# earth-system-radiation/rte-ecckd

Hardware: AMD Instinct MI355X
Metric: Mcol*lay*gpt/s LW gas_optics+rte_lw (higher is better)
Workload: dtype f64

## Files before the change

### rte-ecckd_amd/__init__.py

```python
import ctypes as C
import os
import subprocess

import numpy as np

_HERE = os.path.dirname(os.path.abspath(__file__))
_CSRC = os.path.join(_HERE, "csrc")
LIB_PATH = os.environ.get("ECCKD_LIB", os.path.join(_HERE, "librte_ecckd_hip.so"))
HOST, DEVICE = 0, 1
MIXED = 2
NAME_LEN = 32

_SOURCES = ["kernels_gas_fused.hip", "kernels_tau.hip", "kernels_planck.hip", "kernels_rte_lw.hip", "kernels_rte_lw_split.hip",
            "kernels_rte_lw_jac.hip", "kernels_rte_lw_2str.hip",
            "kernels_rte_sw.hip", "kernels_rte_sw_sys.hip", "kernels_rte_gpt.hip", "kernels_optical_props.hip",
            "kernels_cloud_sampling.hip", "kernels_cloud_optics.hip",
            "capi.cpp", "nc_capi.cpp", "model.cpp", "cdf1.cpp"]
_HEADERS = ["kernels.hpp", "wave_pair.hpp", "sw_two_stream.hpp", "sw_two_stream_body.inc", "lw_two_stream.hpp", "lw_layer.hpp", "planck_at.hpp", "model.hpp", "cdf1.hpp", os.path.join("..", "..", "include", "ecckd_hip.h"),
            os.path.join("..", "..", "include", "ecckd_nc.h"), os.path.join("..", "..", "include", "rte_kernels_hip.h"),
            os.path.join("..", "..", "include", "rte_kernels_lw_2stream_hip.h")]
RTE_KERNELS_LIB = os.path.join(_HERE, "librte_kernels_hip.so")
_RTE_KERNELS_SRC = "rte_kernels_capi.cpp"
HIPCC_FLAGS = ["--offload-arch=gfx950", "-O3", "-std=c++17", "-fPIC", "-shared",
               "-ffp-contract=off", "-Wall", "-Wno-unused-function"]
# ... 189 lines not shown
            getattr(L, f).argtypes = [C.c_void_p, C.c_int, C.c_int] + [C.c_void_p] * 4 + [C.c_int] + [C.c_void_p] * 3 + [C.c_int, C.c_void_p]
    _lib = L
    return L


def last_error():
    return lib().ecckd_last_error().decode()


FAST, REFERENCE_ORDER = 0, 1


def set_arithmetic(mode):
    if lib().ecckd_set_arithmetic(int(mode)):
        raise ValueError(last_error())


def get_arithmetic():
    return lib().ecckd_get_arithmetic()


SOLVER_OPTIONS = ("lw_tau_thresh", "lw_series_terms", "lw_inc_flux_isotropic", "sw_k_floor", "sw_dir_clamp", "lw_solver",
                  "lw_split_seg", "gas_merge_scalars", "lw_tail_split", "sw_tail_split", "sw_solver", "gas_slab_f32",
                  "gas_tile_sync")


def set_solver_option(name, value):
    if lib().ecckd_set_solver_option(name.encode(), float(value)):
        raise ValueError(last_error())


def get_solver_option(name):
    v = C.c_double()
    if lib().ecckd_get_solver_option(name.encode(), C.byref(v)):
        raise ValueError(last_error())
    return v.value


def solver_options():
    out = {}
    for n in SOLVER_OPTIONS:
        try:
            out[n] = get_solver_option(n)
        except ValueError:
            if LIB_PATH == os.path.join(_HERE, "librte_ecckd_hip.so"):
                raise
    return out
# ... 1230 lines not shown
```

### rte-ecckd_amd/csrc/capi.cpp

```cpp
#include <hip/hip_runtime.h>

#include <atomic>
#include <cmath>
#include <cstdint>
#include <cstdlib>
#include <cstring>
#include <map>
#include <mutex>
#include <string>
#include <vector>

#include "../../include/ecckd_hip.h"
#include "kernels.hpp"
#include "model.hpp"

namespace {

thread_local std::string g_err;

int fail(const std::string &msg) {
  g_err = msg;
  return 1;
}
}
// ... 149 lines not shown

double gw(bool f32) {
  return f32 ? (double)(1.f / (9.80665f * 0.001f * 28.970f)) : 1. / ((double)9.80665f * (double)0.001f * (double)28.970f);
}
const double *table(const ecckd_model *m, size_t off, bool f32) {
  return f32 ? reinterpret_cast<const double *>(m->dbuf32 + off) : m->dbuf + off;
}

std::atomic<int> g_arith{0};

struct SolverOptions {
  std::atomic<double> lw_tau_thresh{0.};
  std::atomic<int> lw_series_terms{2};
  std::atomic<int> lw_inc_flux_isotropic{0};
  std::atomic<double> sw_k_floor{1.e-12};
  std::atomic<int> sw_dir_clamp{0};
  std::atomic<int> lw_solver{0};
  std::atomic<int> lw_split_seg{10};
  std::atomic<int> gas_merge_scalars{1};
  std::atomic<int> lw_tail_split{1};
  std::atomic<int> sw_tail_split{1};
  std::atomic<int> gas_slab_f32{2};
  std::atomic<int> gas_tile_sync{-1};
  std::atomic<int> sw_solver{0};
  std::atomic<int> lw_both_skies{1};
  std::atomic<int> lw_jac_inline{1};
};
SolverOptions g_opt;

double lw_tau_thresh(bool f32) {
  const double t = g_opt.lw_tau_thresh.load();
  return t > 0. ? t : (f32 ? std::sqrt(1.1920928955078125e-07) : std::sqrt(2.220446049250313e-16));
}

struct ProfRec { const char *name; hipEvent_t start, stop; };
std::mutex g_prof_mu;
bool g_prof_on = false;
std::vector<ProfRec> g_prof;

struct ProfScope {
  hipStream_t s;
  ProfRec r{};
  bool on;
  ProfScope(const char *name, hipStream_t stream) : s(stream), on(g_prof_on) {
    if (!on) return;
    r.name = name;
    if (hipEventCreate(&r.start) != hipSuccess || hipEventCreate(&r.stop) != hipSuccess) { on = false; return; }
    (void)hipEventRecord(r.start, s);
  }
  ~ProfScope() {
    if (!on) return;
// ... 124 lines not shown
    }
    if (fast) {
      fa.mode = (sw && last) ? 2 : 0;
      if (g_opt.gas_merge_scalars.load() && !f32) merge_scalar_gases(a, f32);
      const int nv_lut = a.lut >= 0 ? a.seq[a.lut].nv : 0;
      int pass_clamp = 0;
      for (int k = 0; k < a.nseq; ++k) pass_clamp |= a.seq[k].clamp;
      if (pl && first_pass && !sw &&
          fused_planck_rows(a.ng, a.np, a.nt, a.nbil, nv_lut, m->ntp, pass_clamp, f32) > 0) {
        fa.mode = 1;
        fa.ntp = m->ntp;
        fa.planck = table(m, m->off_planck, f32);
        fa.pt0 = m->temperature_planck[0];
        fa.pdt = m->temperature_planck[1] - m->temperature_planck[0];
        fa.tlev = pl->tlev; fa.tsfc = pl->tsfc;
        fa.lay_source = pl->lay_source; fa.lev_source_inc = pl->lev_inc;
        fa.lev_source_dec = pl->lev_dec; fa.sfc_source = pl->sfc_source;
        if (planck_done) *planck_done = true;
      }
      fa.f32 = f32;
      {
        const int sync = g_opt.gas_tile_sync.load();
        fa.tile_sync = sync >= 0 ? sync : (fa.mode != 0 ? 1 : 0);
      }
      ScratchLease flag_lease;
      fa.slab32 = (!f32 && !plan && m->f32_exact && fa.mode == 1) ? g_opt.gas_slab_f32.load() : 0;
      if (fa.slab32 == 2) fa.choose_buf = static_cast<int *>(stream_scratch_optional(m->device, stream, 256, flag_lease, g_flag_pool));
      if (f32 && ((fa.mode != 1 && fa.mode != 2) || !last || !first_pass))
        return fail("ecckd: single precision is implemented for one-pass gas optics (fused longwave, shortwave); this "
                    "model / gas list needs the multi-pass or unfused path");
      if (plan) {
        FusedPlan fp;
        HIPCHK(prepare_gas_fused(fa, fp));
        if (plan->npass == 0) { plan->first_fused = 1; plan->planck_fused = fa.mode == 1; plan->first = fp; }
        ++plan->npass;
      } else {
        ProfScope prof(fa.mode == 1 ? (f32 ? "gas_lw_fused_f32" : "gas_lw_fused") : "tau", stream);
        HIPCHK(launch_gas_fused(fa, stream));
      }
    } else {
      if (f32) return fail("ecckd: single precision needs the fast arithmetic mode (ecckd_set_arithmetic(0))");
      if (plan) {
        ++plan->npass;
      } else {
        ProfScope prof("tau", stream);
        HIPCHK(launch_tau(a, stream));
// ... 296 lines not shown
  else if (n == "lw_tail_split") g_opt.lw_tail_split.store(value != 0. ? 1 : 0);
  else if (n == "sw_tail_split") g_opt.sw_tail_split.store(value != 0. ? 1 : 0);
  else if (n == "sw_solver") {
    if (value != 0. && value != 1.) return fail("ecckd_set_solver_option: sw_solver must be 0 (layer-systolic) or 1 (two-pass per lane)");
    g_opt.sw_solver.store((int)value);
  }
  else if (n == "lw_both_skies") {
    if (value != 0. && value != 1.) return fail("ecckd_set_solver_option: lw_both_skies must be 0 (two launches) or 1 (dual-sky kernel)");
    g_opt.lw_both_skies.store((int)value);
  }
  else if (n == "lw_jac_inline") {
    if (value != 0. && value != 1.) return fail("ecckd_set_solver_option: lw_jac_inline must be 0 (stand-alone Jacobian kernel) or 1 (inside the layer-split kernel)");
    g_opt.lw_jac_inline.store((int)value);
  }
  else if (n == "gas_slab_f32") {
    if (value != 0. && value != 1. && value != 2.) return fail("ecckd_set_solver_option: gas_slab_f32 must be 0 (never), 1 (always) or 2 (auto)");
    g_opt.gas_slab_f32.store((int)value);
  }
  else if (n == "gas_tile_sync") {
    if (value != 0. && value != 1. && value != -1.)
      return fail("ecckd_set_solver_option: gas_tile_sync must be 0 (off), 1 (a block barrier per tile) or -1 (the default of each mode)");
    g_opt.gas_tile_sync.store((int)value);
  }
  else return fail("ecckd_set_solver_option: unknown option '" + n + "' (lw_tau_thresh, lw_series_terms, "
                   "lw_inc_flux_isotropic, sw_k_floor, sw_dir_clamp, lw_solver, lw_split_seg, gas_merge_scalars, lw_tail_split, "
                   "sw_tail_split, sw_solver, gas_slab_f32, gas_tile_sync, lw_both_skies, lw_jac_inline)");
  return 0;
}

int ecckd_get_solver_option(const char *name, double *value) {
  if (!name || !value) return fail("ecckd_get_solver_option: null argument");
  const std::string n(name);
  if (n == "lw_tau_thresh") *value = lw_tau_thresh(false);
  else if (n == "lw_series_terms") *value = g_opt.lw_series_terms.load();
  else if (n == "lw_inc_flux_isotropic") *value = g_opt.lw_inc_flux_isotropic.load();
  else if (n == "sw_k_floor") *value = g_opt.sw_k_floor.load();
  else if (n == "sw_dir_clamp") *value = g_opt.sw_dir_clamp.load();
  else if (n == "lw_solver") *value = g_opt.lw_solver.load();
  else if (n == "lw_split_seg") *value = g_opt.lw_split_seg.load();
  else if (n == "gas_merge_scalars") *value = g_opt.gas_merge_scalars.load();
  else if (n == "lw_tail_split") *value = g_opt.lw_tail_split.load();
  else if (n == "sw_tail_split") *value = g_opt.sw_tail_split.load();
  else if (n == "sw_solver") *value = g_opt.sw_solver.load();
  else if (n == "gas_slab_f32") *value = g_opt.gas_slab_f32.load();
  else if (n == "gas_tile_sync") *value = g_opt.gas_tile_sync.load();
  else if (n == "lw_both_skies") *value = g_opt.lw_both_skies.load();
  else if (n == "lw_jac_inline") *value = g_opt.lw_jac_inline.load();
  else return fail("ecckd_get_solver_option: unknown option '" + n + "'");
  return 0;
}

size_t ecckd_rte_lw_scratch_bytes(int ncol, int nlay, int ngpt) {
  return ncol > 0 && nlay > 0 ? ecckd::rte_lw_scratch_bytes(ncol, nlay, ngpt) : 0;
}
size_t ecckd_rte_sw_scratch_bytes(int ncol, int nlay, int ngpt) {
  return ncol > 0 && nlay > 0 ? ecckd::rte_sw_scratch_bytes(ncol, nlay, ngpt) : 0;
}

size_t ecckd_rte_sw_tail_scratch_bytes(int device, int ncol, int nlay, int ngpt) {
  if (ncol <= 0 || nlay <= 0 || ngpt <= 0 || device < 0 || device >= 16 || !g_opt.sw_tail_split.load()) return 0;
  ecckd::RteSwArgs a{};
  a.ncol = ncol; a.nlay = nlay; a.ng = ngpt;
  if (g_opt.sw_solver.load() == 0 && ecckd::rte_sw_sys_applies(a)) return ecckd::rte_sw_sys_plan(a, simd_slots(device) / 4);
  long first = -1;
  size_t at = 0;
  return ecckd::rte_sw_tail_plan(a, &first, &at);
}
static size_t sw_fluxes_solver_bytes(int device, int ncol, int nlay, int ngpt) {
// ... 2118 lines not shown
```

### rte-ecckd_amd/csrc/kernels.hpp

```cpp
#pragma once
#include <hip/hip_runtime.h>

namespace ecckd {

constexpr int kMaxSeq = 16;
constexpr int kTauPassGases = 10;
constexpr int kLdsBudget = 160 * 1024;

struct SeqGas {
  const double *coef;
  const double *vmr;
  long long cs, ls;
  double scalar;
  double ref;
  double mf0;
  double log_mf0;
  double d_log_vmr;
  int code;
  int nv;
  int slot;
  int clamp;
};

struct TauArgs {
// ... 20 lines not shown
  int seg;
};

struct UDiv { double d, r; int exact; };

struct SlotArgs {
  const double *vmr;
  long long ls;
  unsigned cs_bytes;
  double alpha, beta;
};

struct FusedArgs {
  TauArgs tau;
  UDiv ud_dlp, ud_dt, ud_dlv, ud_pdt;
  SlotArgs slot[kTauPassGases + 1];
  int f32;
  int slab32;
  int *choose_buf;
  const int *choose;
  int choose_total;
  int mode;
  int tile_sync;
  int ntp;
  int pw;
  const double *planck;
  double pt0, pdt;
  const double *tlev, *tsfc;
  double *lay_source, *lev_source_inc, *lev_source_dec, *sfc_source;
};

struct PlanckArgs {
  int ncol, nlay, ng, ntp;
  const double *planck;
  double t0, dt;
  const double *tlay, *tlev, *tsfc;
  double *lay_source, *lev_source_inc, *lev_source_dec, *sfc_source;
  int lev_chunks;
};

struct RteLwArgs {
  int ncol, nlay, ng, top_at_1, nmus;
  double Ds[4], wts[4];
  const double *tau, *lay_source, *lev_source_inc, *lev_source_dec, *sfc_source;
  const double *sfc_emis;
  int nband;
// ... 139 lines not shown
};
hipError_t launch_lw_1rescl_gpt(const RteLwRescGptArgs &a, hipStream_t s);

int tau_slab_rows(int ng, int np, int nt, int nbil, int nv_lut);
size_t tau_lds_bytes(int ng, int np, int nt, int nbil, int nv_lut, int R);
size_t rte_lw_scratch_bytes(int ncol, int nlay, int ng);
size_t rte_lw_tail_plan(const RteLwArgs &a, int slots, long *tail_first);
size_t rte_sw_scratch_bytes(int ncol, int nlay, int ng);
size_t rte_sw_tail_plan(const RteSwArgs &a, long *tail_first, size_t *partials_at);

hipError_t launch_tau(TauArgs &a, hipStream_t s);
struct FusedPlan {
  int empty = 0;
  size_t lds_bytes = 0;
  int anyclamp = 0, GC = 0, NB = 0;
  int merged = 0;
  int slab_rows = 0, planck_rows = 0, col_chunks = 0;
};
hipError_t prepare_gas_fused(FusedArgs &a, FusedPlan &plan);
int merge_scalar_gases(TauArgs &t, int f32);
int fused_slab_rows(int ng, int np, int nt, int nbil, int nv_lut, int pl_rows, int min_rows, int anyclamp, int f32, int block = 0);
int fused_planck_rows(int ng, int np, int nt, int nbil, int nv_lut, int ntp, int anyclamp, int f32);
hipError_t launch_gas_fused(FusedArgs &a, hipStream_t s);
hipError_t launch_planck(PlanckArgs &a, hipStream_t s);
hipError_t launch_planck_pair(const PlanckArgs &a, int f32, hipStream_t s);
size_t planck_pair_lds_bytes(int ng, int ntp, int f32);
UDiv make_udiv(double d, int f32);
hipError_t launch_toa_src(const double *solar, int ncol, int ng, double *toa_src, int f32, hipStream_t s);
hipError_t launch_sum_planes(const double *planes, int nplanes, size_t n, double *out, int f32, hipStream_t s);
hipError_t launch_rte_lw(const RteLwArgs &a, hipStream_t s);
bool rte_lw_split_applies(const RteLwArgs &a);
bool rte_lw_planck_fits(int ng, int ntp);
hipError_t launch_rte_lw_split(const RteLwArgs &a, hipStream_t s);
hipError_t launch_rte_lw_planck(const RteLwArgs &a, const double *planck, int ntp, double t0, double dt, const double *tlay,
                                const double *tlev, const double *tsfc, hipStream_t s, double *flux_up_clear = nullptr,
                                double *flux_dn_clear = nullptr, double *flux_up_jac = nullptr);
hipError_t launch_rte_lw_rescaled_split(const RteLwArgs &a, hipStream_t s);
bool rte_lw_rescaled_planck_fits(int ng, int ntp, bool jac = false);
hipError_t launch_rte_lw_rescaled_planck(const RteLwArgs &a, const double *planck, int ntp, double t0, double dt,
                                         const double *tlay, const double *tlev, const double *tsfc, hipStream_t s,
                                         double *flux_up_jac = nullptr);
hipError_t launch_rte_sw(const RteSwArgs &a, hipStream_t s);
bool rte_sw_sys_applies(const RteSwArgs &a);
size_t rte_sw_sys_plan(RteSwArgs &a, int cus);
hipError_t launch_rte_sw_sys(const RteSwArgs &a, int cus, hipStream_t s);
hipError_t launch_rte_sw_tail_reduce(const RteSwArgs &a, int nchunks, int cw, long tail_first, long ntail, hipStream_t s);
// ... 3 lines not shown
```

### rte-ecckd_amd/csrc/kernels_gas_fused.hip

```cpp
#include <cstddef>
#include <cstdlib>
#include <type_traits>

#include "kernels.hpp"
#include "wave_pair.hpp"

namespace ecckd {
namespace {

#ifndef ECCKD_FUSED_BLOCK
#define ECCKD_FUSED_BLOCK 512
#endif
constexpr int kBlock = ECCKD_FUSED_BLOCK;
#ifndef ECCKD_FUSED_BLOCK_SW
#define ECCKD_FUSED_BLOCK_SW 768
#endif
constexpr int kBlockSw = ECCKD_FUSED_BLOCK_SW;
#ifndef ECCKD_FUSED_SEG
#define ECCKD_FUSED_SEG 8
#endif
#ifndef ECCKD_FUSED_SEG_MAX
#define ECCKD_FUSED_SEG_MAX 64
#endif
constexpr int kSeg = ECCKD_FUSED_SEG;
// ... 230 lines not shown
          const int ipl = q % R, itv = q / R;
          const real *src = coef + (long)ng * ((slab_lo + ipl) + (long)np * itv);
          sreal *dst = lds + L.lut + q * L.SL;
          for (int g = lane; g < ng; g += 64) dst[g] = (sreal)src[g];
        }
      }
    };
    const int span = R >= 2 ? R - 1 : 1;
    const int npos = (R >= 2 && ipmin <= ipmax) ? (ipmax - ipmin + span) / span : 1;
    for (int pos = 0; pos < npos; ++pos) {
    const int pos_lo = npos > 1 ? ipmin + pos * span : -0x40000000;
    const int pos_hi = npos > 1 ? pos_lo + span - 1 : 0x40000000;
    if (pos > 0) __syncthreads();
    if (R >= 2 && ipmin <= ipmax) {
      if (npos > 1) {
        const int lo = min(pos_lo - 1, np - R);
        if (lo != slab_lo) stage_slab(lo);
      } else if (!(slab_lo >= 0 && ipmin - 1 >= slab_lo && ipmax <= slab_lo + R - 1)) {
        stage_slab(min(ipmin - 1, np - R));
      }
    }
    __syncthreads();

    real nx_p0, nx_p1, nx_T, nx_W[NB], nx_vlut, nx_Tl0 = real(0), nx_Tl1 = real(0);
    auto load_inputs = [&](long tile) {
      const long c = tile * kBlock + wcol;
      const unsigned cc32 = (unsigned)(c < ncol ? c : (long)ncol - 1);
      const unsigned co = cc32 * (unsigned)sizeof(real);
      auto at = [&](const real *row) { return *reinterpret_cast<greal_t *>((gcchar_t *)row + co); };
      nx_p0 = at(plev0); nx_p1 = at(plev1);
      nx_T = at(P(t.tlay) + (long)ncol * j);
#pragma unroll
      for (int s = 0; s < NB; ++s) nx_W[s] = *reinterpret_cast<greal_t *>(slot_base[s] + cc32 * slot_cs[s]);
      nx_vlut = *reinterpret_cast<greal_t *>(slot_base[NB] + cc32 * slot_cs[NB]);
      if (MODE == MODE_LW && a.tlev) {
        nx_Tl0 = at(P(a.tlev) + (long)ncol * j);
        nx_Tl1 = at(P(a.tlev) + (long)ncol * (j + 1));
      }
    };

    for (long tile = seg; tile < seg_end; ++tile) {
      {
        typedef __attribute__((address_space(4))) const char karg_c;
        typedef __attribute__((address_space(4))) const volatile int karg_i;
        const int tile_sync = *(karg_i *)((karg_c *)__builtin_amdgcn_kernarg_segment_ptr() + offsetof(FusedArgs, tile_sync));
        if (tile_sync) __builtin_amdgcn_s_barrier();
      }
      const long c = tile * kBlock + wcol;
      const bool valid = c < ncol;
      const bool upper = lane >= 32;
      const long cc = c < ncol ? c : (long)ncol - 1;
      load_inputs(tile);
      const real p0 = nx_p0, p1 = nx_p1, Tlayer = nx_T;
      real W[NB];
#pragma unroll
      for (int s = 0; s < NB; ++s) W[s] = nx_W[s];
      real vlut = nx_vlut;
      const real Tl0 = nx_Tl0, Tl1 = nx_Tl1;

      const PPoint<real> pp = pressure_point<real>(p0, p1, lp0, ud_dlp, np);
      const int ip0 = pp.ip0;
      const int ipq = ipmin <= ipmax ? (ip0 < ipmin ? ipmin : (ip0 > ipmax ? ipmax : ip0)) : ip0;
      const bool own = valid && ipq >= pos_lo && ipq <= pos_hi;
      if (!__any(own)) {
        continue;
      }
      const bool lowest = !__any(valid && ipq < pos_lo);
      const bool stray_wave = __any(valid && (ipq != ip0 || ipmin > ipmax));
      int ipl = ip0 - 1 - slab_lo;
      const bool inslab = (R >= 2) && slab_lo >= 0 && ipl >= 0 && ipl + 1 <= R - 1;
      ipl = ipl < 0 ? 0 : (ipl > R - 2 ? (R >= 2 ? R - 2 : 0) : ipl);

      const real t0 = pp.pw0 * (real)lds[L.tb + ip0 - 1] + pp.pw1 * (real)lds[L.tb + ip0];
      real temperature_index = udiv(Tlayer - t0, ud_dt);
      temperature_index = real(1) + selmax(real(0), selmin(temperature_index, (real)nt - real(1.0001)));
      const int it0 = (int)temperature_index;
      const real tw1 = temperature_index - it0;
      const real tw0 = real(1) - tw1;
      const real dp = p1 - p0;
      const real simple_weight = gw * dp;

// ... 2 lines not shown
      int iv0 = 1;
      if (t.lut >= 0) {
        const SeqGas &e = t.seq[t.lut];
        vlut = fma((real)a.slot[kTauPassGases].alpha, vlut, (real)a.slot[kTauPassGases].beta);
        const real log_vmr = log(selmax(vlut, (real)e.mf0));
        real vmr_index = udiv(log_vmr - (real)e.log_mf0, ud_dlv);
        vmr_index = real(1) + selmax(real(0), selmin(vmr_index, (real)e.nv - real(1.001)));
        iv0 = (int)vmr_index;
        const real vw1 = vmr_index - iv0, vw0 = real(1) - vw1;
        real wl = simple_weight * vlut;
        if (!ANYCLAMP) wl = wl < real(0) ? real(0) : wl;
        const real u0 = ANYCLAMP ? vw0 : wl * vw0, u1 = ANYCLAMP ? vw1 : wl * vw1;
        l000 = u0 * a00; l100 = u0 * a10; l010 = u0 * a01; l110 = u0 * a11;
        l001 = u1 * a00; l101 = u1 * a10; l011 = u1 * a01; l111 = u1 * a11;
        if (ANYCLAMP) vlut = wl;
      }
#pragma unroll
      for (int s = 0; s < NB; ++s) {
        const SlotArgs &e = a.slot[s];
        real x = simple_weight * fma((real)e.alpha, W[s], (real)e.beta);
        if (!ANYCLAMP) x = x < real(0) ? real(0) : x;
        W[s] = x;
      }
      PlPoint<real> qlay{0, 0, real(0), real(0)}, ql0{0, 0, real(0), real(0)}, ql1{0, 0, real(0), real(0)};
      bool inwin = true;
      if (MODE == MODE_LW) {
        qlay = planck_point<real>(Tlayer, pt0, ud_pdt, ntp);
        ql0 = (a.tlev && j == 0) ? planck_point<real>(Tl0, pt0, ud_pdt, ntp) : qlay;
        ql1 = a.tlev ? planck_point<real>(Tl1, pt0, ud_pdt, ntp) : qlay;
        const int rmin = min(qlay.row, min(ql0.row, ql1.row)), rmax = max(qlay.row, max(ql0.row, ql1.row));
        inwin = rmin >= pw_lo && rmax + 1 <= pw_lo + PW - 1;
        qlay.off = (qlay.row - pw_lo) * L.SP;
        ql0.off = (ql0.row - pw_lo) * L.SP;
        ql1.off = (ql1.row - pw_lo) * L.SP;
      }
      const real moles = dp * gw;
      const bool slow_wave = __any(valid && !(inwin && R >= 2 && slab_lo >= 0)) || stray_wave;
      const bool fast = !slow_wave;
      const bool active = own && inslab;
      const bool masked_wave = !__all(active);
      const bool mine = slow_wave ? (lowest && valid) : active;
      const int ip0_ = ip0, it0_ = it0, iv0_ = iv0;

      if (fast) {
        static_assert(GC % 4 == 0, "chunks are made of g-point pairs");
        constexpr int NP2 = GC / 2;
        constexpr int NLI = 2 * NP2, NBI = NB * NP2;
        const int ob = L.bil + (ipl + R * (it0 - 1)) * L.SB;
        const int ol = t.lut >= 0 ? L.lut + (ipl + R * ((it0 - 1) + nt * (iv0 - 1))) * L.SL : L.bil;
        const int dPb = L.SB, dTb = R * L.SB;
        const int dPl = t.lut >= 0 ? L.SL : 0, dTl = t.lut >= 0 ? R * L.SL : 0, dVl = t.lut >= 0 ? R * nt * L.SL : 0;
        constexpr int ES = (int)sizeof(sreal);
        int ab[4] = {ES * ob, ES * (ob + dPb), ES * (ob + dTb), ES * (ob + dTb + dPb)};
        int al[8] = {ES * ol, ES * (ol + dPl), ES * (ol + dTl), ES * (ol + dTl + dPl),
                     ES * (ol + dVl), ES * (ol + dVl + dPl), ES * (ol + dVl + dTl), ES * (ol + dVl + dTl + dPl)};
        int ap[6] = {ES * (L.pl + qlay.off), ES * (L.pl + qlay.off + L.SP), ES * (L.pl + ql1.off), ES * (L.pl + ql1.off + L.SP),
                     ES * (L.pl + ql0.off), ES * (L.pl + ql0.off + L.SP)};
        const int cstride = ES * t.nbil * GC;
        const unsigned plane = (unsigned)ncol * (unsigned)nlay;
        const unsigned coff = (unsigned)sizeof(real) * (unsigned)cc;
        const unsigned voff = (unsigned)sizeof(real) * ((unsigned)(c - (upper ? 1 : 0)) + (upper ? plane : 0u));
        const long plane2 = 2L * plane;
        real *w_tau = Q(t.tau) + (long)ncol * j, *w_ssa = MODE == MODE_SW && t.ssa ? Q(t.ssa) + (long)ncol * j : nullptr;
        real *w_g = MODE == MODE_SW && t.ssa ? Q(t.g) + (long)ncol * j : nullptr;
        real *w_lay = MODE == MODE_LW ? Q(a.lay_source) + (long)ncol * j : nullptr;
        const bool has_next = j + 1 < nlay;
        real *w_dec0 = MODE == MODE_LW && a.tlev ? Q(a.lev_source_dec) + (long)ncol * j : nullptr;
        real *w_decn = MODE == MODE_LW && a.tlev ? Q(a.lev_source_dec) + (long)ncol * (j + 1) : nullptr;
        real *w_inc = MODE == MODE_LW && a.tlev ? Q(a.lev_source_inc) + (long)ncol * j : nullptr;
        auto chunks = [&](auto masked_c, auto first_c) __attribute__((always_inline)) {
        constexpr bool masked = decltype(masked_c)::value;
        constexpr bool FIRST = decltype(first_c)::value;
        constexpr int NPI = (MODE == MODE_LW) ? (FIRST ? 2 * NP2 : NP2) : 0;
        constexpr int NIT = NLI + NBI + NPI;
        for (int gb = 0; gb < ngp; gb += GC) {
          real acc[GC];
          if (MODE != MODE_LW && t.accumulate) {
            typedef __attribute__((address_space(1))) const char gcchar;
            typedef __attribute__((address_space(1))) const real greal;
#pragma unroll
            for (int g = 0; g < GC; ++g) {
              acc[g] = real(0);
              if (FULL || gb + g < ng) {
                gcchar *pl = (gcchar *)(P(t.tau) + (long)ncol * (j + (long)nlay * (gb + g)));
                asm volatile("" : "+s"(pl));
                acc[g] = *reinterpret_cast<greal *>(pl + coff);
              }
            }
          } else {
#pragma unroll
            for (int g = 0; g < GC; ++g) acc[g] = real(0);
          }
          asm volatile("" : "+v"(ab[0]), "+v"(ab[1]), "+v"(ab[2]), "+v"(ab[3]));
          asm volatile("" : "+v"(al[0]), "+v"(al[1]), "+v"(al[2]), "+v"(al[3]), "+v"(al[4]), "+v"(al[5]), "+v"(al[6]), "+v"(al[7]));
          if (MODE == MODE_LW) asm volatile("" : "+v"(ap[0]), "+v"(ap[1]), "+v"(ap[2]), "+v"(ap[3]));
          if (MODE == MODE_LW && FIRST) asm volatile("" : "+v"(ap[4]), "+v"(ap[5]));
          double2_t buf[2][4];
          real lutp[2] = {real(0), real(0)};
          static_for<0, NIT + 1>([&](auto pos_c) __attribute__((always_inline)) {
            constexpr int pos = decltype(pos_c)::value;
            constexpr int it = pos < NIT ? seq_item(pos, NLI, NBI, NPI) : NIT;
            if constexpr (it < NLI) {
              constexpr int g = 2 * (it / 2), h = it & 1;
              double2_t *b = buf[pos & 1];
              b[0] = ld2b(al[4 * h], g); b[1] = ld2b(al[4 * h + 1], g); b[2] = ld2b(al[4 * h + 2], g); b[3] = ld2b(al[4 * h + 3], g);
            } else if constexpr (it < NLI + NBI) {
              constexpr int so = bil_slot(it - NLI, NP2) * GC + 2 * bil_pair(it - NLI, NP2);
              double2_t *b = buf[pos & 1];
              b[0] = ld2b(ab[0], so); b[1] = ld2b(ab[1], so); b[2] = ld2b(ab[2], so); b[3] = ld2b(ab[3], so);
            } else if constexpr (it < NIT) {
              constexpr int k = it - NLI - NBI;
              double2_t *b = buf[pos & 1];
              if constexpr (k < NP2) {
                constexpr int g = 2 * k;
                b[0] = ld2b(ap[0], g); b[1] = ld2b(ap[1], g);
                b[2] = ld2b(ap[2], g); b[3] = ld2b(ap[3], g);
              } else {
                constexpr int g = 2 * (k - NP2);
                b[0] = ld2b(ap[4], g); b[1] = ld2b(ap[5], g);
              }
            }
            if constexpr (pos >= 1) {
              constexpr int pi_ = seq_item(pos - 1, NLI, NBI, NPI);
              const double2_t *b = buf[(pos - 1) & 1];
              if constexpr (pi_ < NLI) {
                const int g0 = 2 * (pi_ / 2);
                if ((pi_ & 1) == 0) {
#pragma unroll
                  for (int q = 0; q < 2; ++q) {
                    real v = l000 * (real)b[0][q];
                    v = fma(l100, (real)b[1][q], v); v = fma(l010, (real)b[2][q], v); v = fma(l110, (real)b[3][q], v);
                    asm volatile("" : "+v"(v));
                    lutp[q] = v;
                  }
                } else {
#pragma unroll
                  for (int q = 0; q < 2; ++q) {
                    real v = lutp[q];
                    v = fma(l001, (real)b[0][q], v); v = fma(l101, (real)b[1][q], v); v = fma(l011, (real)b[2][q], v);
                    v = fma(l111, (real)b[3][q], v);
                    if (ANYCLAMP) { v = vlut * v; v = v < real(0) ? real(0) : v; }
                    acc[g0 + q] = acc[g0 + q] + v;
                    asm volatile("" : "+v"(acc[g0 + q]));
// ... 9 lines not shown
                  else acc[g0 + q] = fma(W[s], v, acc[g0 + q]);
                  asm volatile("" : "+v"(acc[g0 + q]));
                }
                if (pi_ == NLI + NBI - 1) {
#pragma unroll
                  for (int g = 0; g < GC; g += 2) {
                    const int npl = FULL ? 2 : ng - (gb + g);
                    if (FULL || npl >= 1) {
                      if (MODE == MODE_SW) {
                        const real r0 = moles * P(t.rayleigh)[gb + g], r1 = moles * P(t.rayleigh)[gb + g + 1];
                        const real t0_ = acc[g] + r0, t1_ = acc[g + 1] + r1;
                        store_pair<real>(w_tau, plane2, voff, coff, t0_, t1_, masked, active, npl, upper);
                        if (t.ssa) {
                          store_pair<real>(w_ssa, plane2, voff, coff, r0 / t0_, r1 / t1_, masked, active, npl, upper);
                          store_pair<real>(w_g, plane2, voff, coff, real(0), real(0), masked, active, npl, upper);
                        }
                      } else {
                        store_pair<real>(w_tau, plane2, voff, coff, acc[g], acc[g + 1], masked, active, npl, upper);
                      }
                    }
                  }
                }
              } else {
                constexpr int k = pi_ - NLI - NBI;
                constexpr int g = 2 * (k < NP2 ? k : k - NP2);
                const int npl = FULL ? 2 : ng - (gb + g);
                if constexpr (k < NP2) {
                  real vl[2], v1[2];
#pragma unroll
                  for (int q = 0; q < 2; ++q) {
                    vl[q] = div_pi(qlay.w0 * (real)b[0][q] + qlay.w1 * (real)b[1][q], pi, rpi);
                    v1[q] = div_pi(ql1.w0 * (real)b[2][q] + ql1.w1 * (real)b[3][q], pi, rpi);
                  }
                  if (FULL || npl >= 1) {
                    store_pair<real>(w_lay, plane2, voff, coff, vl[0], vl[1], masked, active, npl, upper);
                    if (a.tlev) {
                      store_pair<real>(w_inc, plane2, voff, coff, v1[0], v1[1], masked, active, npl, upper);
                      if (has_next) store_pair<real>(w_decn, plane2, voff, coff, v1[0], v1[1], masked, active, npl, upper);
                    }
                  }
                } else {
                  real v0[2];
#pragma unroll
                  for (int q = 0; q < 2; ++q) v0[q] = div_pi(ql0.w0 * (real)b[0][q] + ql0.w1 * (real)b[1][q], pi, rpi);
                  if (a.tlev && (FULL || npl >= 1)) store_pair<real>(w_dec0, plane2, voff, coff, v0[0], v0[1], masked, active, npl, upper);
                }
              }
            }
          });
#pragma unroll
          for (int q = 0; q < 4; ++q) ab[q] += cstride;
#pragma unroll
          for (int q = 0; q < 8; ++q) al[q] += ES * GC;
#pragma unroll
          for (int q = 0; q < 6; ++q) ap[q] += ES * GC;
        }
        };
        if (j == 0) {
          if (masked_wave) chunks(std::true_type{}, std::true_type{}); else chunks(std::false_type{}, std::true_type{});
        } else {
          if (masked_wave) chunks(std::true_type{}, std::false_type{}); else chunks(std::false_type{}, std::false_type{});
        }
      } else if (lowest) {
        int ip0 = ip0_, it0 = it0_, iv0 = iv0_;
        asm volatile("" : "+v"(ip0), "+v"(it0), "+v"(iv0));
        for (int g = 0; g < ng; ++g) {
          const long o = cc + (long)ncol * (j + (long)nlay * g);
          real acc = t.accumulate ? P(t.tau)[o] : real(0);
          if (t.lut >= 0) {
            const SeqGas &e = t.seq[t.lut];
            const real *cp = P(e.coef) + (long)ng * ((ip0 - 1) + (long)np * ((it0 - 1) + (long)nt * (iv0 - 1))) + g;
            const long dP = ng, dT = (long)ng * np, dV = (long)ng * np * nt;
            real v = l000 * cp[0];
            v = fma(l100, cp[dP], v);
            v = fma(l010, cp[dT], v);
            v = fma(l110, cp[dT + dP], v);
            v = fma(l001, cp[dV], v);
            v = fma(l101, cp[dV + dP], v);
            v = fma(l011, cp[dV + dT], v);
            v = fma(l111, cp[dV + dT + dP], v);
            if (ANYCLAMP) { v = vlut * v; v = v < real(0) ? real(0) : v; }
            acc = acc + v;
          }
#pragma unroll
          for (int s = 0; s < NB; ++s) {
// ... 11 lines not shown
              v = fma(a10, c10, v);
              v = fma(a01, c01, v);
              v = fma(a11, c11, v);
              if (ANYCLAMP) { v = W[s] * v; v = v < real(0) ? real(0) : v; acc = acc + v; }
              else acc = fma(W[s], v, acc);
            }
          }
          if (valid) {
            if (MODE == MODE_SW) {
              const real ray = moles * P(t.rayleigh)[g];
              const real tt = acc + ray;
              Q(t.tau)[o] = tt;
              if (t.ssa) { Q(t.ssa)[o] = ray / tt; Q(t.g)[o] = real(0); }
            } else {
              Q(t.tau)[o] = acc;
            }
            if (MODE == MODE_LW) {
              const real *pg = P(a.planck) + g;
              Q(a.lay_source)[o] = div_pi(qlay.w0 * pg[(long)qlay.row * ng] + qlay.w1 * pg[(long)(qlay.row + 1) * ng], pi, rpi);
              if (a.tlev) {
                const real v1 = div_pi(ql1.w0 * pg[(long)ql1.row * ng] + ql1.w1 * pg[(long)(ql1.row + 1) * ng], pi, rpi);
                Q(a.lev_source_inc)[o] = v1;
                if (j + 1 < nlay) Q(a.lev_source_dec)[o + ncol] = v1;
                if (j == 0)
                  Q(a.lev_source_dec)[o] = div_pi(ql0.w0 * pg[(long)ql0.row * ng] + ql0.w1 * pg[(long)(ql0.row + 1) * ng], pi, rpi);
              }
            }
          }
        }
      }

      if (MODE == MODE_LW && j == 0 && mine) {
        const PlPoint<real> qs = planck_point<real>(P(a.tsfc)[c], pt0, ud_pdt, ntp);
        const real *p0r = P(a.planck) + (long)qs.row * ng, *p1r = p0r + ng;
        for (int g = 0; g < ng; ++g)
          Q(a.sfc_source)[c + (long)ncol * g] = div_pi(qs.w0 * p0r[g] + qs.w1 * p1r[g], pi, rpi);
      }
    }
    }
  }
}

template <typename real, int GC, int NB, bool FULL, bool ANYCLAMP, int MODE, typename sreal = real>
hipError_t launch_one(const FusedArgs &a, size_t lds_bytes, hipStream_t s) {
  constexpr int kBlock = fused_block(MODE);
  auto k = gas_fused_kernel<real, GC, NB, FULL, ANYCLAMP, MODE, sreal, kBlock>;
  hipError_t e = hipFuncSetAttribute(reinterpret_cast<const void *>(k),
                                     hipFuncAttributeMaxDynamicSharedMemorySize, (int)lds_bytes);
  if (e != hipSuccess) return e;
  hipLaunchKernelGGL(k, dim3(a.tau.col_chunks, a.tau.nlay), dim3(kBlock), lds_bytes, s, a);
  return hipGetLastError();
}

int pick_nb(int nbil) {
  if (nbil <= 2) return 2;
  if (nbil <= 5) return 5;
  if (nbil <= 7) return 7;
  return kTauPassGases;
}
// ... 161 lines not shown
  t.R = fused_slab_rows(t.ng, t.np, t.nt, t.nbil, nv_lut, a.pw, 0, anyclamp, store, block);
  const size_t lds = (store ? sizeof(float) : sizeof(double)) *
                     (size_t)f_layout(ngp, t.np, t.nt, t.nbil, NB, nv_lut, t.R, a.pw, store == 2 ? 2 : 1, block / 64).total;
  if (lds > (size_t)kLdsBudget) return hipErrorInvalidValue;
  const long ntiles = ((long)t.ncol + block - 1) / block;
  long chunks = 1;
  while ((chunks * t.nlay) % 256 != 0 && chunks < 256) ++chunks;
  while (chunks * 2 * kSeg <= ntiles && chunks * t.nlay < 2048) chunks *= 2;
  if (chunks * kSeg > ntiles) chunks = (ntiles + kSeg - 1) / kSeg;
  if (chunks < 1) chunks = 1;
  t.col_chunks = (int)chunks;
  {
    long per_block = (ntiles + chunks - 1) / chunks;
    t.seg = (int)(per_block < kSeg ? kSeg : (per_block > kSegMax ? kSegMax : per_block));
  }
  if (a.f32 && a.mode == MODE_TAU) return hipErrorNotSupported;
  plan.lds_bytes = lds;
  plan.anyclamp = anyclamp ? 1 : 0;
  plan.GC = GC; plan.NB = NB; plan.merged = t.merge_slot >= 0 ? t.nmerge : 0;
  plan.slab_rows = t.R; plan.planck_rows = a.pw; plan.col_chunks = t.col_chunks;
  return hipSuccess;
}

hipError_t launch_gas_fused(FusedArgs &a, hipStream_t s) {
  FusedPlan plan;
  if (a.slab32 == 2) {
    FusedArgs b = a;
    b.slab32 = 1;
    FusedPlan pb;
    hipError_t eb = prepare_gas_fused(b, pb);
    if (eb == hipSuccess && !pb.empty && b.slab32 == 1 && a.choose_buf) {
      a.slab32 = 0;
      eb = prepare_gas_fused(a, plan);
      if (eb != hipSuccess) return eb;
      const TauArgs &t = a.tau;
      eb = hipMemsetAsync(a.choose_buf, 0, sizeof(int), s);
      if (eb != hipSuccess) return eb;
      const long nw = ((long)t.ncol + 63) / 64;
      hipLaunchKernelGGL(spread_probe_kernel<double>, dim3((unsigned)((t.ncol + 255) / 256), t.nlay > 1 ? 2 : 1), dim3(256), 0, s,
                         t.plev, t.ncol, t.nlay, t.lp0, a.ud_dlp, t.np, a.choose_buf);
      eb = hipGetLastError();
      if (eb != hipSuccess) return eb;
      a.choose = b.choose = a.choose_buf;
      a.choose_total = b.choose_total = (int)(nw > 0x7fffffff ? 0x7fffffff : nw);
      eb = launch_mode<double, MODE_LW>(a, plan.lds_bytes, pick_nb(t.nbil), plan.anyclamp != 0, s);
      if (eb != hipSuccess) return eb;
      return launch_one<double, 8, 7, true, false, MODE_LW, float>(b, pb.lds_bytes, s);
    }
    a.slab32 = 0;
  }
  const hipError_t e = prepare_gas_fused(a, plan);
  if (e != hipSuccess || plan.empty) return e;
  const TauArgs &t = a.tau;
  const bool anyclamp = plan.anyclamp != 0;
  if (a.slab32 && !a.f32) return launch_one<double, 8, 7, true, false, MODE_LW, float>(a, plan.lds_bytes, s);
  if (a.f32 && a.mode == MODE_SW) return launch_mode<float, MODE_SW>(a, plan.lds_bytes, pick_nb(t.nbil), anyclamp, s);
  if (a.f32) return launch_mode<float, MODE_LW>(a, plan.lds_bytes, pick_nb(t.nbil), anyclamp, s);
  if (a.mode == MODE_LW) return launch_mode<double, MODE_LW>(a, plan.lds_bytes, pick_nb(t.nbil), anyclamp, s);
  if (a.mode == MODE_SW) return launch_mode<double, MODE_SW>(a, plan.lds_bytes, pick_nb(t.nbil), anyclamp, s);
  return launch_mode<double, MODE_TAU>(a, plan.lds_bytes, pick_nb(t.nbil), anyclamp, s);
}

}
```

### rte-ecckd_amd/csrc/kernels_planck.hip

```cpp
#include "kernels.hpp"
#include "wave_pair.hpp"

namespace ecckd {
namespace {

constexpr int kPlBlock = 512;

__device__ __forceinline__ double div_pi(double x, double pi, double rpi) {
  const double q = x * rpi;
  const double r = fma(-q, pi, x);
  return fma(r, rpi, q);
}

struct PlanckPoint {
  int row;
  double w0, w1;
  bool below;
};

__device__ __forceinline__ PlanckPoint planck_point(double T, double t0, double dt, int ntp) {
  PlanckPoint p;
  double temperature_index = (T - t0) / dt;
  if (temperature_index >= 0) {
    temperature_index = 1. + temperature_index;
// ... 175 lines not shown
        w_inc[c] = v1;
        if (has_next) w_dec[c] = v1;
      }
    }
    if (j == 0) {
      const PlPoint<real> q0 = planck_point<real>(((greal *)P(a.tlev))[cc], t0, ud_dt, ntp);
      int a0 = q0.row * SP * ES;
      real *w_dec0 = Q(a.lev_source_dec);
      for (int p = 0; p < npairs; ++p, a0 += 2 * ES) {
        real v0[2];
        interp(q0, a0, 0, v0);
        store_pair<real>(w_dec0, plane2, voff, coff, v0[0], v0[1], masked, valid);
      }
      if ((ng & 1) && valid) w_dec0[c] = single(q0, a0, 0);
    }
  }
  if (blockIdx.y == 0 && valid) {
    const PlPoint<real> qs = planck_point<real>(P(a.tsfc)[c], t0, ud_dt, ntp);
    const int as = qs.row * SP * ES;
    for (int g = 0; g < ng; ++g) Q(a.sfc_source)[c + (long)ncol * g] = single(qs, as, g);
  }
}

}

size_t planck_pair_lds_bytes(int ng, int ntp, int f32) {
  return (f32 ? sizeof(float) : sizeof(double)) * (size_t)ntp * row_stride(ng + (ng & 1));
}

hipError_t launch_planck_pair(const PlanckArgs &a, int f32, hipStream_t s) {
  if (a.ncol <= 0) return hipSuccess;
  const size_t lds = planck_pair_lds_bytes(a.ng, a.ntp, f32);
  if (lds > (size_t)kLdsBudget) return hipErrorInvalidValue;
  if (((size_t)a.ncol * (size_t)a.nlay + (size_t)a.ncol) * (f32 ? sizeof(float) : sizeof(double)) >= (size_t)0xFFFFFFF0u)
    return hipErrorInvalidValue;
  const int nb = (a.ncol + kPpBlock - 1) / kPpBlock;
  int chunks = 1;
  while (chunks < 6 && (long)nb * chunks < 4096 && (chunks + 1) * 4 <= a.nlay) ++chunks;
  const UDiv ud = make_udiv(a.dt, f32);
  hipError_t e;
  auto go = [&](auto k) {
    e = hipFuncSetAttribute(reinterpret_cast<const void *>(k), hipFuncAttributeMaxDynamicSharedMemorySize, (int)lds);
    if (e != hipSuccess) return e;
    hipLaunchKernelGGL(k, dim3(nb, chunks), dim3(kPpBlock), lds, s, a, ud);
    return hipGetLastError();
  };
// ... 21 lines not shown
```

Baseline: 84440.

## Prefetch next tile inputs and move edge Planck sources to separate kernel

```diff
diff --git a/rte-ecckd_amd/__init__.py b/rte-ecckd_amd/__init__.py
--- a/rte-ecckd_amd/__init__.py
+++ b/rte-ecckd_amd/__init__.py
@@ -235,7 +235,7 @@
 
 SOLVER_OPTIONS = ("lw_tau_thresh", "lw_series_terms", "lw_inc_flux_isotropic", "sw_k_floor", "sw_dir_clamp", "lw_solver",
                   "lw_split_seg", "gas_merge_scalars", "lw_tail_split", "sw_tail_split", "sw_solver", "gas_slab_f32",
-                  "gas_tile_sync")
+                  "gas_tile_sync", "gas_input_ahead")
 
 
 def set_solver_option(name, value):
diff --git a/rte-ecckd_amd/csrc/capi.cpp b/rte-ecckd_amd/csrc/capi.cpp
--- a/rte-ecckd_amd/csrc/capi.cpp
+++ b/rte-ecckd_amd/csrc/capi.cpp
@@ -195,11 +195,13 @@
   std::atomic<int> sw_tail_split{1};
   std::atomic<int> gas_slab_f32{2};
   std::atomic<int> gas_tile_sync{-1};
+  std::atomic<int> gas_input_ahead{-1};
   std::atomic<int> sw_solver{0};
   std::atomic<int> lw_both_skies{1};
   std::atomic<int> lw_jac_inline{1};
 };
 SolverOptions g_opt;
+constexpr int kGasInputAheadDefault[2] = {1, 0};
 
 double lw_tau_thresh(bool f32) {
   const double t = g_opt.lw_tau_thresh.load();
@@ -370,6 +372,8 @@
       {
         const int sync = g_opt.gas_tile_sync.load();
         fa.tile_sync = sync >= 0 ? sync : (fa.mode != 0 ? 1 : 0);
+        const int ahead = g_opt.gas_input_ahead.load();
+        fa.input_ahead = ahead >= 0 ? ahead : kGasInputAheadDefault[f32 ? 1 : 0];
       }
       ScratchLease flag_lease;
       fa.slab32 = (!f32 && !plan && m->f32_exact && fa.mode == 1) ? g_opt.gas_slab_f32.load() : 0;
@@ -712,9 +716,14 @@
       return fail("ecckd_set_solver_option: gas_tile_sync must be 0 (off), 1 (a block barrier per tile) or -1 (the default of each mode)");
     g_opt.gas_tile_sync.store((int)value);
   }
+  else if (n == "gas_input_ahead") {
+    if (value != 0. && value != 1. && value != -1.)
+      return fail("ecckd_set_solver_option: gas_input_ahead must be 0 (inputs loaded at the top of a tile), 1 (a tile ahead) or -1 (the default of each mode)");
+    g_opt.gas_input_ahead.store((int)value);
+  }
   else return fail("ecckd_set_solver_option: unknown option '" + n + "' (lw_tau_thresh, lw_series_terms, "
                    "lw_inc_flux_isotropic, sw_k_floor, sw_dir_clamp, lw_solver, lw_split_seg, gas_merge_scalars, lw_tail_split, "
-                   "sw_tail_split, sw_solver, gas_slab_f32, gas_tile_sync, lw_both_skies, lw_jac_inline)");
+                   "sw_tail_split, sw_solver, gas_slab_f32, gas_tile_sync, gas_input_ahead, lw_both_skies, lw_jac_inline)");
   return 0;
 }
 
@@ -734,6 +743,7 @@
   else if (n == "sw_solver") *value = g_opt.sw_solver.load();
   else if (n == "gas_slab_f32") *value = g_opt.gas_slab_f32.load();
   else if (n == "gas_tile_sync") *value = g_opt.gas_tile_sync.load();
+  else if (n == "gas_input_ahead") *value = g_opt.gas_input_ahead.load();
   else if (n == "lw_both_skies") *value = g_opt.lw_both_skies.load();
   else if (n == "lw_jac_inline") *value = g_opt.lw_jac_inline.load();
   else return fail("ecckd_get_solver_option: unknown option '" + n + "'");
diff --git a/rte-ecckd_amd/csrc/kernels.hpp b/rte-ecckd_amd/csrc/kernels.hpp
--- a/rte-ecckd_amd/csrc/kernels.hpp
+++ b/rte-ecckd_amd/csrc/kernels.hpp
@@ -66,6 +66,7 @@
   int choose_total;
   int mode;
   int tile_sync;
+  int input_ahead;
   int ntp;
   int pw;
   const double *planck;
@@ -251,6 +252,7 @@
 int fused_slab_rows(int ng, int np, int nt, int nbil, int nv_lut, int pl_rows, int min_rows, int anyclamp, int f32, int block = 0);
 int fused_planck_rows(int ng, int np, int nt, int nbil, int nv_lut, int ntp, int anyclamp, int f32);
 hipError_t launch_gas_fused(FusedArgs &a, hipStream_t s);
+hipError_t launch_planck_edge(const FusedArgs &a, hipStream_t s);
 hipError_t launch_planck(PlanckArgs &a, hipStream_t s);
 hipError_t launch_planck_pair(const PlanckArgs &a, int f32, hipStream_t s);
 size_t planck_pair_lds_bytes(int ng, int ntp, int f32);
diff --git a/rte-ecckd_amd/csrc/kernels_gas_fused.hip b/rte-ecckd_amd/csrc/kernels_gas_fused.hip
--- a/rte-ecckd_amd/csrc/kernels_gas_fused.hip
+++ b/rte-ecckd_amd/csrc/kernels_gas_fused.hip
@@ -276,7 +276,9 @@
     }
     __syncthreads();
 
-    real nx_p0, nx_p1, nx_T, nx_W[NB], nx_vlut, nx_Tl0 = real(0), nx_Tl1 = real(0);
+    constexpr bool kAhead = BLOCK == 512;
+    real nx_p0, nx_p1, nx_T, nx_W[NB], nx_vlut, nx_Tl1 = real(0);
+    bool nx_loaded = false;
     auto load_inputs = [&](long tile) {
       const long c = tile * kBlock + wcol;
       const unsigned cc32 = (unsigned)(c < ncol ? c : (long)ncol - 1);
@@ -287,16 +289,13 @@
 #pragma unroll
       for (int s = 0; s < NB; ++s) nx_W[s] = *reinterpret_cast<greal_t *>(slot_base[s] + cc32 * slot_cs[s]);
       nx_vlut = *reinterpret_cast<greal_t *>(slot_base[NB] + cc32 * slot_cs[NB]);
-      if (MODE == MODE_LW && a.tlev) {
-        nx_Tl0 = at(P(a.tlev) + (long)ncol * j);
-        nx_Tl1 = at(P(a.tlev) + (long)ncol * (j + 1));
-      }
+      if (MODE == MODE_LW && a.tlev) nx_Tl1 = at(P(a.tlev) + (long)ncol * (j + 1));
     };
 
     for (long tile = seg; tile < seg_end; ++tile) {
+      typedef __attribute__((address_space(4))) const char karg_c;
+      typedef __attribute__((address_space(4))) const volatile int karg_i;
       {
-        typedef __attribute__((address_space(4))) const char karg_c;
-        typedef __attribute__((address_space(4))) const volatile int karg_i;
         const int tile_sync = *(karg_i *)((karg_c *)__builtin_amdgcn_kernarg_segment_ptr() + offsetof(FusedArgs, tile_sync));
         if (tile_sync) __builtin_amdgcn_s_barrier();
       }
@@ -304,13 +303,14 @@
       const bool valid = c < ncol;
       const bool upper = lane >= 32;
       const long cc = c < ncol ? c : (long)ncol - 1;
-      load_inputs(tile);
+      if (!(kAhead && nx_loaded)) load_inputs(tile);
+      nx_loaded = false;
       const real p0 = nx_p0, p1 = nx_p1, Tlayer = nx_T;
       real W[NB];
 #pragma unroll
       for (int s = 0; s < NB; ++s) W[s] = nx_W[s];
       real vlut = nx_vlut;
-      const real Tl0 = nx_Tl0, Tl1 = nx_Tl1;
+      const real Tl1 = nx_Tl1;
 
       const PPoint<real> pp = pressure_point<real>(p0, p1, lp0, ud_dlp, np);
       const int ip0 = pp.ip0;
@@ -359,16 +359,14 @@
         if (!ANYCLAMP) x = x < real(0) ? real(0) : x;
         W[s] = x;
       }
-      PlPoint<real> qlay{0, 0, real(0), real(0)}, ql0{0, 0, real(0), real(0)}, ql1{0, 0, real(0), real(0)};
+      PlPoint<real> qlay{0, 0, real(0), real(0)}, ql1{0, 0, real(0), real(0)};
       bool inwin = true;
       if (MODE == MODE_LW) {
         qlay = planck_point<real>(Tlayer, pt0, ud_pdt, ntp);
-        ql0 = (a.tlev && j == 0) ? planck_point<real>(Tl0, pt0, ud_pdt, ntp) : qlay;
         ql1 = a.tlev ? planck_point<real>(Tl1, pt0, ud_pdt, ntp) : qlay;
-        const int rmin = min(qlay.row, min(ql0.row, ql1.row)), rmax = max(qlay.row, max(ql0.row, ql1.row));
+        const int rmin = min(qlay.row, ql1.row), rmax = max(qlay.row, ql1.row);
         inwin = rmin >= pw_lo && rmax + 1 <= pw_lo + PW - 1;
         qlay.off = (qlay.row - pw_lo) * L.SP;
-        ql0.off = (ql0.row - pw_lo) * L.SP;
         ql1.off = (ql1.row - pw_lo) * L.SP;
       }
       const real moles = dp * gw;
@@ -376,8 +374,15 @@
       const bool fast = !slow_wave;
       const bool active = own && inslab;
       const bool masked_wave = !__all(active);
-      const bool mine = slow_wave ? (lowest && valid) : active;
       const int ip0_ = ip0, it0_ = it0, iv0_ = iv0;
+
+      if (kAhead) {
+        const int ahead = *(karg_i *)((karg_c *)__builtin_amdgcn_kernarg_segment_ptr() + offsetof(FusedArgs, input_ahead));
+        if (ahead) {
+          load_inputs(tile + 1);
+          nx_loaded = true;
+        }
+      }
 
       if (fast) {
         static_assert(GC % 4 == 0, "chunks are made of g-point pairs");
@@ -391,8 +396,7 @@
         int ab[4] = {ES * ob, ES * (ob + dPb), ES * (ob + dTb), ES * (ob + dTb + dPb)};
         int al[8] = {ES * ol, ES * (ol + dPl), ES * (ol + dTl), ES * (ol + dTl + dPl),
                      ES * (ol + dVl), ES * (ol + dVl + dPl), ES * (ol + dVl + dTl), ES * (ol + dVl + dTl + dPl)};
-        int ap[6] = {ES * (L.pl + qlay.off), ES * (L.pl + qlay.off + L.SP), ES * (L.pl + ql1.off), ES * (L.pl + ql1.off + L.SP),
-                     ES * (L.pl + ql0.off), ES * (L.pl + ql0.off + L.SP)};
+        int ap[4] = {ES * (L.pl + qlay.off), ES * (L.pl + qlay.off + L.SP), ES * (L.pl + ql1.off), ES * (L.pl + ql1.off + L.SP)};
         const int cstride = ES * t.nbil * GC;
         const unsigned plane = (unsigned)ncol * (unsigned)nlay;
         const unsigned coff = (unsigned)sizeof(real) * (unsigned)cc;
@@ -402,13 +406,11 @@
         real *w_g = MODE == MODE_SW && t.ssa ? Q(t.g) + (long)ncol * j : nullptr;
         real *w_lay = MODE == MODE_LW ? Q(a.lay_source) + (long)ncol * j : nullptr;
         const bool has_next = j + 1 < nlay;
-        real *w_dec0 = MODE == MODE_LW && a.tlev ? Q(a.lev_source_dec) + (long)ncol * j : nullptr;
         real *w_decn = MODE == MODE_LW && a.tlev ? Q(a.lev_source_dec) + (long)ncol * (j + 1) : nullptr;
         real *w_inc = MODE == MODE_LW && a.tlev ? Q(a.lev_source_inc) + (long)ncol * j : nullptr;
-        auto chunks = [&](auto masked_c, auto first_c) __attribute__((always_inline)) {
+        auto chunks = [&](auto masked_c) __attribute__((always_inline)) {
         constexpr bool masked = decltype(masked_c)::value;
-        constexpr bool FIRST = decltype(first_c)::value;
-        constexpr int NPI = (MODE == MODE_LW) ? (FIRST ? 2 * NP2 : NP2) : 0;
+        constexpr int NPI = (MODE == MODE_LW) ? NP2 : 0;
         constexpr int NIT = NLI + NBI + NPI;
         for (int gb = 0; gb < ngp; gb += GC) {
           real acc[GC];
@@ -431,7 +433,6 @@
           asm volatile("" : "+v"(ab[0]), "+v"(ab[1]), "+v"(ab[2]), "+v"(ab[3]));
           asm volatile("" : "+v"(al[0]), "+v"(al[1]), "+v"(al[2]), "+v"(al[3]), "+v"(al[4]), "+v"(al[5]), "+v"(al[6]), "+v"(al[7]));
           if (MODE == MODE_LW) asm volatile("" : "+v"(ap[0]), "+v"(ap[1]), "+v"(ap[2]), "+v"(ap[3]));
-          if (MODE == MODE_LW && FIRST) asm volatile("" : "+v"(ap[4]), "+v"(ap[5]));
           double2_t buf[2][4];
           real lutp[2] = {real(0), real(0)};
           static_for<0, NIT + 1>([&](auto pos_c) __attribute__((always_inline)) {
@@ -446,16 +447,10 @@
               double2_t *b = buf[pos & 1];
               b[0] = ld2b(ab[0], so); b[1] = ld2b(ab[1], so); b[2] = ld2b(ab[2], so); b[3] = ld2b(ab[3], so);
             } else if constexpr (it < NIT) {
-              constexpr int k = it - NLI - NBI;
+              constexpr int g = 2 * (it - NLI - NBI);
               double2_t *b = buf[pos & 1];
-              if constexpr (k < NP2) {
-                constexpr int g = 2 * k;
-                b[0] = ld2b(ap[0], g); b[1] = ld2b(ap[1], g);
-                b[2] = ld2b(ap[2], g); b[3] = ld2b(ap[3], g);
-              } else {
-                constexpr int g = 2 * (k - NP2);
-                b[0] = ld2b(ap[4], g); b[1] = ld2b(ap[5], g);
-              }
+              b[0] = ld2b(ap[0], g); b[1] = ld2b(ap[1], g);
+              b[2] = ld2b(ap[2], g); b[3] = ld2b(ap[3], g);
             }
             if constexpr (pos >= 1) {
               constexpr int pi_ = seq_item(pos - 1, NLI, NBI, NPI);
@@ -511,28 +506,20 @@
                   }
                 }
               } else {
-                constexpr int k = pi_ - NLI - NBI;
-                constexpr int g = 2 * (k < NP2 ? k : k - NP2);
+                constexpr int g = 2 * (pi_ - NLI - NBI);
                 const int npl = FULL ? 2 : ng - (gb + g);
-                if constexpr (k < NP2) {
-                  real vl[2], v1[2];
-#pragma unroll
-                  for (int q = 0; q < 2; ++q) {
-                    vl[q] = div_pi(qlay.w0 * (real)b[0][q] + qlay.w1 * (real)b[1][q], pi, rpi);
-                    v1[q] = div_pi(ql1.w0 * (real)b[2][q] + ql1.w1 * (real)b[3][q], pi, rpi);
+                real vl[2], v1[2];
+#pragma unroll
+                for (int q = 0; q < 2; ++q) {
+                  vl[q] = div_pi(qlay.w0 * (real)b[0][q] + qlay.w1 * (real)b[1][q], pi, rpi);
+                  v1[q] = div_pi(ql1.w0 * (real)b[2][q] + ql1.w1 * (real)b[3][q], pi, rpi);
+                }
+                if (FULL || npl >= 1) {
+                  store_pair<real>(w_lay, plane2, voff, coff, vl[0], vl[1], masked, active, npl, upper);
+                  if (a.tlev) {
+                    store_pair<real>(w_inc, plane2, voff, coff, v1[0], v1[1], masked, active, npl, upper);
+                    if (has_next) store_pair<real>(w_decn, plane2, voff, coff, v1[0], v1[1], masked, active, npl, upper);
                   }
-                  if (FULL || npl >= 1) {
-                    store_pair<real>(w_lay, plane2, voff, coff, vl[0], vl[1], masked, active, npl, upper);
-                    if (a.tlev) {
-                      store_pair<real>(w_inc, plane2, voff, coff, v1[0], v1[1], masked, active, npl, upper);
-                      if (has_next) store_pair<real>(w_decn, plane2, voff, coff, v1[0], v1[1], masked, active, npl, upper);
-                    }
-                  }
-                } else {
-                  real v0[2];
-#pragma unroll
-                  for (int q = 0; q < 2; ++q) v0[q] = div_pi(ql0.w0 * (real)b[0][q] + ql0.w1 * (real)b[1][q], pi, rpi);
-                  if (a.tlev && (FULL || npl >= 1)) store_pair<real>(w_dec0, plane2, voff, coff, v0[0], v0[1], masked, active, npl, upper);
                 }
               }
             }
@@ -542,14 +529,10 @@
 #pragma unroll
           for (int q = 0; q < 8; ++q) al[q] += ES * GC;
 #pragma unroll
-          for (int q = 0; q < 6; ++q) ap[q] += ES * GC;
+          for (int q = 0; q < 4; ++q) ap[q] += ES * GC;
         }
         };
-        if (j == 0) {
-          if (masked_wave) chunks(std::true_type{}, std::true_type{}); else chunks(std::false_type{}, std::true_type{});
-        } else {
-          if (masked_wave) chunks(std::true_type{}, std::false_type{}); else chunks(std::false_type{}, std::false_type{});
-        }
+        if (masked_wave) chunks(std::true_type{}); else chunks(std::false_type{});
       } else if (lowest) {
         int ip0 = ip0_, it0 = it0_, iv0 = iv0_;
         asm volatile("" : "+v"(ip0), "+v"(it0), "+v"(iv0));
@@ -607,19 +590,10 @@
                 const real v1 = div_pi(ql1.w0 * pg[(long)ql1.row * ng] + ql1.w1 * pg[(long)(ql1.row + 1) * ng], pi, rpi);
                 Q(a.lev_source_inc)[o] = v1;
                 if (j + 1 < nlay) Q(a.lev_source_dec)[o + ncol] = v1;
-                if (j == 0)
-                  Q(a.lev_source_dec)[o] = div_pi(ql0.w0 * pg[(long)ql0.row * ng] + ql0.w1 * pg[(long)(ql0.row + 1) * ng], pi, rpi);
               }
             }
           }
         }
-      }
-
-      if (MODE == MODE_LW && j == 0 && mine) {
-        const PlPoint<real> qs = planck_point<real>(P(a.tsfc)[c], pt0, ud_pdt, ntp);
-        const real *p0r = P(a.planck) + (long)qs.row * ng, *p1r = p0r + ng;
-        for (int g = 0; g < ng; ++g)
-          Q(a.sfc_source)[c + (long)ncol * g] = div_pi(qs.w0 * p0r[g] + qs.w1 * p1r[g], pi, rpi);
       }
     }
     }
@@ -827,7 +801,18 @@
   return hipSuccess;
 }
 
+namespace {
+hipError_t launch_gas_fused_layers(FusedArgs &a, hipStream_t s);
+}
+
 hipError_t launch_gas_fused(FusedArgs &a, hipStream_t s) {
+  const hipError_t e = launch_gas_fused_layers(a, s);
+  if (e != hipSuccess || a.mode != MODE_LW) return e;
+  return launch_planck_edge(a, s);
+}
+
+namespace {
+hipError_t launch_gas_fused_layers(FusedArgs &a, hipStream_t s) {
   FusedPlan plan;
   if (a.slab32 == 2) {
     FusedArgs b = a;
@@ -865,5 +850,6 @@
   if (a.mode == MODE_SW) return launch_mode<double, MODE_SW>(a, plan.lds_bytes, pick_nb(t.nbil), anyclamp, s);
   return launch_mode<double, MODE_TAU>(a, plan.lds_bytes, pick_nb(t.nbil), anyclamp, s);
 }
-
-}
+}
+
+}
diff --git a/rte-ecckd_amd/csrc/kernels_planck.hip b/rte-ecckd_amd/csrc/kernels_planck.hip
--- a/rte-ecckd_amd/csrc/kernels_planck.hip
+++ b/rte-ecckd_amd/csrc/kernels_planck.hip
@@ -221,6 +221,59 @@
   }
 }
 
+constexpr int kPeBlock = 256;
+constexpr int kPeGroup = 8;
+
+template <typename real>
+__global__ void __launch_bounds__(kPeBlock) planck_edge_kernel(const real *planck, int ng, int ntp, real t0, const UDiv ud_dt_h, int ncol,
+                                                               int nlay, const real *tsfc, const real *tlev, real *sfc_source,
+                                                               real *lev_source_dec) {
+  typedef real real2_u __attribute__((ext_vector_type(2), aligned(sizeof(real))));
+  const long c = (long)blockIdx.x * kPeBlock + threadIdx.x;
+  if (c >= ncol) return;
+  const bool top = blockIdx.y != 0;
+  const UDivT<real> ud_dt = make_udiv_t<real>(ud_dt_h);
+  const real pi = (real)3.14159265359f, rpi = real(1) / pi;
+  const PlPoint<real> q = planck_point<real>(top ? tlev[c] : tsfc[c], t0, ud_dt, ntp);
+  const real *p0r = planck + (long)q.row * ng, *p1r = p0r + ng;
+  real *out = (top ? lev_source_dec : sfc_source) + c;
+  const long plane = top ? (long)ncol * nlay : (long)ncol;
+  const int g0 = blockIdx.z * kPeGroup, g1 = g0 + kPeGroup < ng ? g0 + kPeGroup : ng;
+  real2_u b0[kPeGroup / 2], b1[kPeGroup / 2];
+#pragma unroll
+  for (int p = 0; p < kPeGroup / 2; ++p) {
+    const int g = g0 + 2 * p;
+    if (g + 1 < g1) {
+      b0[p] = *reinterpret_cast<const real2_u *>(p0r + g);
+      b1[p] = *reinterpret_cast<const real2_u *>(p1r + g);
+    } else if (g < g1) {
+      b0[p][0] = p0r[g]; b0[p][1] = real(0);
+      b1[p][0] = p1r[g]; b1[p][1] = real(0);
+    }
+  }
+#pragma unroll
+  for (int p = 0; p < kPeGroup / 2; ++p) {
+    const int g = g0 + 2 * p;
+    if (g < g1) __builtin_nontemporal_store(div_pi(q.w0 * b0[p][0] + q.w1 * b1[p][0], pi, rpi), out + plane * g);
+    if (g + 1 < g1) __builtin_nontemporal_store(div_pi(q.w0 * b0[p][1] + q.w1 * b1[p][1], pi, rpi), out + plane * (g + 1));
+  }
+}
+
+}
+
+hipError_t launch_planck_edge(const FusedArgs &a, hipStream_t s) {
+  const TauArgs &t = a.tau;
+  if (t.ncol <= 0 || t.nlay <= 0) return hipSuccess;
+  const dim3 grid((unsigned)((t.ncol + kPeBlock - 1) / kPeBlock), a.tlev ? 2 : 1, (unsigned)((t.ng + kPeGroup - 1) / kPeGroup));
+  if (a.f32)
+    hipLaunchKernelGGL(planck_edge_kernel<float>, grid, dim3(kPeBlock), 0, s, reinterpret_cast<const float *>(a.planck), t.ng, a.ntp,
+                       (float)a.pt0, a.ud_pdt, t.ncol, t.nlay, reinterpret_cast<const float *>(a.tsfc),
+                       reinterpret_cast<const float *>(a.tlev), reinterpret_cast<float *>(a.sfc_source),
+                       reinterpret_cast<float *>(a.lev_source_dec));
+  else
+    hipLaunchKernelGGL(planck_edge_kernel<double>, grid, dim3(kPeBlock), 0, s, a.planck, t.ng, a.ntp, a.pt0, a.ud_pdt, t.ncol, t.nlay,
+                       a.tsfc, a.tlev, a.sfc_source, a.lev_source_dec);
+  return hipGetLastError();
 }
 
 size_t planck_pair_lds_bytes(int ng, int ntp, int f32) {
```

Result: faster. 85380, median of 6 (+1.1%).
